# harvardinformatics/IMCoalHMM

Measured on AMD Instinct MI355X. Metric: alignment columns/sec (forward pass), 20-state isolation HMM, higher is better.
Workload: dtype f64

## Files before the change

imcoalhmm_amd/csrc/imcoal_fwd.hip:

```cpp
#include <hip/hip_runtime.h>

#include <algorithm>
#include <cerrno>
#include <climits>
#include <cmath>
#include <cstdint>
#include <cstdio>
#include <cstdlib>
#include <cstring>
#include <list>
#include <atomic>
#include <chrono>
#include <map>
#include <set>
#include <memory>
#include <mutex>
#include <condition_variable>
#include <string>
#include <vector>

#include <unistd.h>

#include "../../include/imcoal_fwd.h"
#include "kernels_plain.hpp"
// ... 35 lines not shown
constexpr size_t DICT_TRAIN_MIN = 32768;
constexpr size_t DICT_TRAIN_MAX = 8u << 20;
constexpr size_t DICT_WIDE_TRAIN_TOKENS = 1u << 19;
constexpr int DICT_MAX_DEPTH = 0;
constexpr size_t DICT_WIDE_MIN_COUNT = 6;
constexpr size_t CTAB_BUDGET = (size_t)24 << 30;
#ifndef IMC_HYBRID_MAX_ALPHABET
#define IMC_HYBRID_MAX_ALPHABET 4096
#endif
constexpr int HYBRID_MAX_ALPHABET = IMC_HYBRID_MAX_ALPHABET;
constexpr size_t Z2GRAN = 4;
constexpr size_t R1_MIN_SEGLEN = 1024;
constexpr size_t R1_MIN_HEAD = 256;
constexpr double R1_HEAD_COLUMNS = 65536.0;
constexpr double R1_HEAD_MIN_COLUMNS = 8192.0;
constexpr int R1_MAX_ROUNDS = 24;
constexpr double R1_DENSE_COLUMNS = 1.0e5;

hipError_t dev_alloc(void **p, size_t bytes);
void dev_free(void *p);

struct DictDev {
    imc::PairDict dict;
    uint16_t *d_left = nullptr, *d_right = nullptr;
    uint16_t *d_order = nullptr;
    std::vector<uint16_t> order;
    std::vector<int> depth;
    uint64_t trained_on = 0;
    pid_t pid = 0;
    ~DictDev()
    {
        if (pid == getpid()) { dev_free(d_left); dev_free(d_right); dev_free(d_order); }
    }
};

struct Ev3 { hipEvent_t a, b, c; };

struct Ctx {
    pid_t pid = 0;
    int device = -1;
    bool ready = false;
    hipStream_t stream = nullptr;
    int cus = 256;
    uint64_t next_obs_id = 1, next_dict_id = 1;
    size_t seg_override = 0;
    int compression = 1;
    int kernel_pref = 0;
    bool profile = false;
    bool rank1_handoff = true;
    int blocked_variant = 4;
    int z4_stream = -1;
    bool table_pairs = true;
    int table_triples = -1;
    bool xcd_affine = true;
    int fuse_tail = 1;
    bool fuse_head = true;
    bool pack_table = true;
    bool guard = false;
    bool use_graphs = false;
    std::vector<Ev3> events;
    std::map<int, std::shared_ptr<DictDev>> dicts;
    uint64_t last_plan[8] = {0, 0, 0, 0, 0, 0, 0, 0};
    uint64_t r1_checked = 0, r1_collapsed = 0;
    std::string last_kernels;
} g;

void drop_plans();
void reset_kernel_attributes();

int ensure_ctx()
{
    const pid_t me = getpid();
    if (g.ready && g.pid == me) return IMC_OK;
    if (g.ready && g.pid != me)
        return fail(IMC_ERR_HIP, "libimcoal_fwd was initialised in the parent process before fork(): fork the chain "
                                 "processes before the first imc_* call of the parent, or use the spawn start method");
    int n = 0;
    if (hipGetDeviceCount(&n) != hipSuccess || n <= 0)
        return fail(IMC_ERR_NODEVICE, "no HIP device available (libimcoal_fwd has no CPU fallback)");
    if (g.device < 0) {
        int cur = 0;
        if (hipGetDevice(&cur) != hipSuccess) cur = 0;
        g.device = cur;
    }
    if (g.device >= n) return fail(IMC_ERR_NODEVICE, "requested device index out of range");
    HIP_TRY(hipSetDevice(g.device));
    hipDeviceProp_t prop;
    HIP_TRY(hipGetDeviceProperties(&prop, g.device));
    if (std::strncmp(prop.gcnArchName, "gfx950", 6) != 0)
        return fail(IMC_ERR_NODEVICE, std::string("device is ") + prop.gcnArchName + ", this library is built for gfx950 only");
    g.cus = prop.multiProcessorCount > 0 ? prop.multiProcessorCount : 256;
    HIP_TRY(hipStreamCreateWithFlags(&g.stream, hipStreamNonBlocking));
    g.use_graphs = std::getenv("IMC_GRAPH") != nullptr;
    if (const char *gd = std::getenv("IMC_GUARD")) g.guard = std::atoi(gd) != 0;
    if (const char *bv = std::getenv("IMC_BLOCKED")) { const int v = std::atoi(bv); if (v >= 2 && v <= 5) g.blocked_variant = v; }
    if (const char *r1 = std::getenv("IMC_RANK1")) g.rank1_handoff = std::atoi(r1) != 0;
    if (const char *pt = std::getenv("IMC_PACK_TABLE")) g.pack_table = std::atoi(pt) != 0;
    if (const char *tp = std::getenv("IMC_TABLE_PAIRS")) g.table_pairs = std::atoi(tp) != 0;
    if (const char *fh = std::getenv("IMC_FUSE_HEAD")) g.fuse_head = std::atoi(fh) != 0;
    if (const char *tt = std::getenv("IMC_TABLE_TRIPLES")) g.table_triples = std::atoi(tt) != 0 ? 1 : 0;
    if (const char *ft = std::getenv("IMC_FUSE_TAIL")) g.fuse_tail = std::max(0, std::min(2, std::atoi(ft)));
    if (const char *xa = std::getenv("IMC_XCD_AFFINE")) g.xcd_affine = std::atoi(xa) != 0;
    if (const char *zs = std::getenv("IMC_Z4_STREAM")) { const int v = std::atoi(zs); if (v >= -1 && v <= 1) g.z4_stream = v; }
    g.pid = me;
    g.ready = true;
    return IMC_OK;
}

struct GuardRec { hipDeviceptr_t va; size_t va_size; hipMemGenericAllocationHandle_t handle; hipDeviceptr_t map; size_t map_size; };
std::map<void *, GuardRec> &g_guard = *new std::map<void *, GuardRec>();

hipError_t dev_alloc(void **p, size_t bytes)
{
    bytes = std::max<size_t>(bytes, 16);
    if (!g.guard) return hipMalloc(p, bytes);
    hipMemAllocationProp prop{};
    prop.type = hipMemAllocationTypePinned;
    prop.location.type = hipMemLocationTypeDevice;
    prop.location.id = g.device;
    size_t gran = 0;
    hipError_t e = hipMemGetAllocationGranularity(&gran, &prop, hipMemAllocationGranularityMinimum);
    if (e != hipSuccess || gran == 0) return e != hipSuccess ? e : hipErrorUnknown;
    GuardRec r{};
    r.map_size = (bytes + gran - 1) / gran * gran;
    r.va_size = r.map_size + 2 * gran;
    e = hipMemAddressReserve(&r.va, r.va_size, gran, nullptr, 0);
    if (e != hipSuccess) return e;
    e = hipMemCreate(&r.handle, r.map_size, &prop, 0);
    if (e != hipSuccess) { (void)hipMemAddressFree(r.va, r.va_size); return e; }
    r.map = (hipDeviceptr_t)((char *)r.va + gran);
    e = hipMemMap(r.map, r.map_size, 0, r.handle, 0);
    if (e == hipSuccess) {
        hipMemAccessDesc ad{};
        ad.location = prop.location;
        ad.flags = hipMemAccessFlagsProtReadWrite;
        e = hipMemSetAccess(r.map, r.map_size, &ad, 1);
        if (e != hipSuccess) (void)hipMemUnmap(r.map, r.map_size);
    }
    if (e != hipSuccess) { (void)hipMemRelease(r.handle); (void)hipMemAddressFree(r.va, r.va_size); return e; }
    void *user = (char *)r.map + (r.map_size - (bytes + 15) / 16 * 16);
    g_guard[user] = r;
    *p = user;
    return hipSuccess;
}

void dev_free(void *p)
{
    if (!p) return;
    auto it = g_guard.find(p);
    if (it == g_guard.end()) { (void)hipFree(p); return; }
    (void)hipDeviceSynchronize();
    (void)hipMemUnmap(it->second.map, it->second.map_size);
// ... 183 lines not shown
    for (int l = 0; l < imc::kNumLevels; ++l) { o->d_tok[l] = nullptr; o->wide[l] = false; o->ntok[l] = 0; o->alphabet[l] = nsym; }
    hipError_t e = wide_raw ? upload_padded(reinterpret_cast<const uint8_t *>(host16), L * sizeof(imc::tok_t), &o->d_sym)
                            : upload_padded(host, L, &o->d_sym);
    if (e != hipSuccess) {
        delete o;
        return fail(e == hipErrorOutOfMemory ? IMC_ERR_OOM : IMC_ERR_HIP,
                    std::string("observation upload: ") + hipGetErrorString(e));
    }
    if (zipped) {
        if (int rc = install_encoding(o, dd, enc)) {
            obs_release(o);
            delete o;
            return rc;
        }
    }
    *out = o;
    return IMC_OK;
}


using ChainFn = void (*)(const ChainDesc *, int, const uint32_t *, uint32_t, uint32_t, const double *, const int *,
                         const int *, uint32_t, double *, int *, double *, int);

struct KernelChoice {
    int R, G, NP, VPW, minw;
    void (*plain)(PropArgs);
    void (*zip)(PropArgs);
    size_t (*zip_lds)(int);
    ChainFn chain;
    bool zip_attr_set;
    void (*big_table_raw)(BigArgs);
    void (*big_table_level)(BigArgs, const uint16_t *, int);
    void (*big_prop)(BigArgs, const BigBlock *);
    int big_prop_waves;
    void (*big_vec)(BigArgs, const BigBlock *, int, int);
    void (*big_vec_tail)(BigArgs, const BigBlock *, int, int);
    int big_vec_waves;
    int big_nslab;
    size_t big_lds;
    void (*zip2)(BigArgs);
    size_t (*zip2_lds)(int);
    bool zip2_attr_set;
    bool plain_attr_set = false;
    void (*zip3)(BigArgs) = nullptr;
    size_t (*zip3_lds)(int) = nullptr;
    bool zip3_attr_set = false;
    void (*zip4)(BigArgs) = nullptr;
    void (*zip4w)(BigArgs) = nullptr;
    void (*zip4s)(BigArgs) = nullptr, (*zip4sw)(BigArgs) = nullptr;
    void (*zip4_raw)(BigArgs) = nullptr;
    void (*zip4_level)(BigArgs, int, int) = nullptr;
    void (*zip4_level2)(BigArgs, const int4 *, int, int, const double *) = nullptr;
    void (*zip4_level2_first)(BigArgs, const int4 *, int, int, const double *) = nullptr;
    void (*zip4_level3)(BigArgs, const int4 *, int, int, const double *) = nullptr;
    void (*zip4_level3_first)(BigArgs, const int4 *, int, int, const double *) = nullptr;
    size_t (*zip4_level3_lds)(size_t) = nullptr;
    size_t (*zip4_lds)(int, int) = nullptr;
    int (*zip4_max_hot)(int, size_t) = nullptr;
    int tok_doubles = 0;
    bool chain_self_emax = false;
    bool zip4_attr_set = false, zip4w_attr_set = false, zip4s_attr_set = false, zip4sw_attr_set = false, zip4_attr_l3 = false;
    bool use3() const;
    size_t blocked_lds(int A) const { return use3() ? zip3_lds(A) : zip2_lds(A); }
};

template <int R, int G, int MW>
KernelChoice make_kc()
{
    constexpr int NP = R * G;
    KernelChoice k{R, G, NP, 64 / G, MW, k_propagate<R, G, MW>, k_zpropagate<R, G>, &ZipGeom<R, G>::lds_bytes,
                   k_chain<NP, (NP <= 12 ? 6 : NP <= 24 ? 4 : NP <= 32 ? 3 : NP <= 64 ? 2 : 1)>, false, nullptr, nullptr, nullptr, 0, nullptr, nullptr, 0, 0, 0, nullptr, nullptr, false};
    k.chain_self_emax = true;
    if constexpr (NP % 4 == 0 && NP <= 24) {
        k.zip2 = k_zpropagate2<NP / 4>;
        k.zip2_lds = &Zip2Geom<NP / 4>::lds_bytes;
        k.zip3 = k_zpropagate3<NP / 4>;
        k.zip3_lds = &Zip3Geom<NP / 4>::lds_bytes;
        k.tok_doubles = Zip3Geom<NP / 4>::TOK;
        if constexpr (NP <= 24) {
            k.zip4 = k_zpropagate4<NP / 4, false, true>;
            k.zip4w = k_zpropagate4<NP / 4, true, true>;
            k.zip4s = k_zpropagate4<NP / 4, false, false>;
            k.zip4sw = k_zpropagate4<NP / 4, true, false>;
            k.zip4_raw = k_z4_raw<NP / 4>;
            k.zip4_level = k_z4_level<NP / 4>;
            k.zip4_level2 = k_z4_level2<NP / 4, false>;
            k.zip4_level2_first = k_z4_level2<NP / 4, true>;
            k.zip4_level3 = k_z4_level3<NP / 4, false>;
            k.zip4_level3_first = k_z4_level3<NP / 4, true>;
            k.zip4_level3_lds = &Z4L3Geom<NP / 4>::lds_bytes;
            k.zip4_lds = &Zip4Geom<NP / 4>::lds_bytes;
            k.zip4_max_hot = &Zip4Geom<NP / 4>::max_hot;
        }
    }
    return k;
}

template <int NT, int NSLAB>
KernelChoice make_big()
{
    constexpr int NP = 16 * NT;
    constexpr bool dealt = NT > 4 && NT % 4 != 0;
    void (*prop)(BigArgs, const BigBlock *) = k_big_propagate<NT, NSLAB>;
    if constexpr (dealt) prop = k_big_propagate_s<NT, NSLAB>;
    return KernelChoice{0, NT, NP, 0, 1, nullptr, nullptr, nullptr, k_chain<NP, 0>, false, k_big_table_raw<NT>,
                        k_big_table_level<NT>, prop, dealt ? BS_WAVES : NT, k_big_vector<NT, false>, k_big_vector<NT, true>, BigVec<NT>::WAVES, NSLAB,
                        BigSlab<NT, NSLAB>::bytes, nullptr, nullptr, false};
}

bool KernelChoice::use3() const { return zip3 && g.blocked_variant >= 3; }

KernelChoice kChoices[] = {
    make_kc<4, 1, 2>(), make_kc<4, 2, 2>(), make_kc<4, 3, 2>(), make_kc<4, 4, 2>(), make_kc<4, 5, 2>(),
    make_kc<3, 8, 2>(), make_kc<2, 14, 2>(), make_kc<2, 16, 2>(), make_kc<2, 20, 1>(), make_kc<1, 48, 1>(),
    make_kc<1, 56, 1>(), make_kc<1, 64, 1>(),
    make_big<6, 1>(), make_big<7, 1>(), make_big<8, 2>(), make_big<9, 3>(), make_big<10, 2>(), make_big<12, 3>(), make_big<14, 7>(),
    make_big<16, 8>(),
};
constexpr int IMC_MAX_N = 256;

KernelChoice kMidChoices[] = {make_big<2, 1>(), make_big<3, 1>(), make_big<4, 1>()};

KernelChoice *choose_kernel(int N, bool prefer_gemm)
{
    if (prefer_gemm && N > 24 && N <= 64)
        for (auto &k : kMidChoices)
            if (k.NP >= N) return &k;
    for (auto &k : kChoices)
        if (k.NP >= N) return &k;
    return nullptr;
}

void reset_kernel_attributes()
{
    for (auto &k : kChoices) k.zip4_attr_l3 = k.zip_attr_set = k.zip2_attr_set = k.zip3_attr_set = k.zip4_attr_set = k.zip4w_attr_set = k.zip4s_attr_set = k.zip4sw_attr_set = k.plain_attr_set = false;
    for (auto &k : kMidChoices) k.zip4_attr_l3 = k.zip_attr_set = k.zip2_attr_set = k.zip3_attr_set = k.zip4_attr_set = k.zip4w_attr_set = k.zip4s_attr_set = k.zip4sw_attr_set = k.plain_attr_set = false;
}


struct Group {
// ... 937 lines not shown
    for (int b = 0; b < B; ++b) {
        double *pp = p->h_params[p->slot] + (size_t)b * p->pstride;
        std::memset(pp, 0, p->pstride * 8);
        const double *pi = pis + (size_t)b * N, *T = Ts + (size_t)b * N * N, *E = Es + (size_t)b * N * S;
        for (int i = 0; i < N; ++i) pp[i] = pi[i];
        double *Tp = pp + NP;
        for (int j = 0; j < N; ++j) std::memcpy(Tp + (size_t)j * NP, T + (size_t)j * N, (size_t)N * 8);
        double *Et = pp + NP + (size_t)NP * NP;
        for (int s = 0; s < S; ++s)
            for (int i = 0; i < N; ++i) Et[(size_t)s * NP + i] = E[(size_t)i * S + s];
    }
    return IMC_OK;
}

int enqueue(Plan *p, hipStream_t stream, double *out, bool allow_tail = true)
{
    KernelChoice *kc = p->kc;
    const int N = p->N, S = p->S, NP = kc->NP, B = p->B;
    hipStreamCaptureStatus cap = hipStreamCaptureStatusNone;
    (void)hipStreamIsCapturing(stream, &cap);
    if (cap == hipStreamCaptureStatusNone && p->have_last && p->last_stream != stream)
        HIP_TRY(hipStreamWaitEvent(stream, p->ev_params[p->last_slot], 0));
    const size_t pbytes = (size_t)B * p->pstride * 8;
    bool fuse_head = false, direct_params = false;
    {
        int active = 0;
        const Group *only = nullptr;
        for (const Group &gr : p->groups)
            if (gr.n_vecs) { ++active; only = &gr; }
        const size_t head_lds = p->pstride * 8;
        fuse_head = g.fuse_head && active == 1 && only->zip4 && g.table_pairs && only->d_tab_desc2 && !only->tab2.empty() &&
                    kc->zip4_level2_first && pbytes <= STAGE_KERNEL_MAX_BYTES && head_lds <= 16 * 1024;
        direct_params = g.fuse_head && active == 1 && only->zip2 && !only->zip4 && kc->use3() && pbytes <= STAGE_KERNEL_MAX_BYTES &&
                        only->blocks.size() * (size_t)B <= 32 && p->pstride * 8 <= 8192 &&
                        ((kc->blocked_lds(only->A) + 15) & ~(size_t)15) + p->pstride * 8 <= LDS_BUDGET;
    }
    if (fuse_head || direct_params) {
    } else if (pbytes <= STAGE_KERNEL_MAX_BYTES) {
        const unsigned n2 = (unsigned)(pbytes / 16);
        hipLaunchKernelGGL(k_stage_params, dim3((n2 + 255) / 256), dim3(256), 0, stream,
                           reinterpret_cast<const double2 *>(p->h_params_dev[p->slot]), reinterpret_cast<double2 *>(p->d_params), n2);
        HIP_TRY(hipGetLastError());
    } else {
        HIP_TRY(hipMemcpyAsync(p->d_params, p->h_params[p->slot], pbytes, hipMemcpyHostToDevice, stream));
    }

    uint64_t *lp = p->lp;
    lp[0] = p->n_segs; lp[1] = p->n_vecs; lp[2] = lp[3] = lp[4] = lp[5] = lp[6] = lp[7] = 0;
    Ev3 ev{nullptr, nullptr, nullptr};
    const bool prof = g.profile && p->n_vecs;
    bool a_recorded = false;
    if (prof) { HIP_TRY(hipEventCreate(&ev.a)); HIP_TRY(hipEventCreate(&ev.b)); HIP_TRY(hipEventCreate(&ev.c)); }
#define IMC_MARK_A() do { if (prof && !a_recorded) { HIP_TRY(hipEventRecord(ev.a, stream)); a_recorded = true; } } while (0)
    bool tail_used = false;
    p->kernels.clear();
    auto note = [&](const std::string &k) { p->kernels += (p->kernels.empty() ? "" : "+") + k; };
    for (const Group &gr : p->groups) {
        if (!gr.n_vecs) continue;
        if (!gr.zip4) IMC_MARK_A();
        const std::string strm = gr.zip ? "[tokens]" : "[columns]";
        PropArgs a;
        a.segs = p->d_segs; a.vecs = p->d_vecs + gr.vec_begin; a.n_vecs = gr.n_vecs; a.vec_base = gr.vec_begin;
        a.n_vecs_total = p->n_vecs; a.N = N; a.S = S;
        a.params = p->d_params; a.pstride = p->pstride; a.P = p->levels[0].d_P; a.EX = p->levels[0].d_EX;
        a.A = gr.A; a.tok_left = gr.zip ? gr.dict->d_left : nullptr; a.tok_right = gr.zip ? gr.dict->d_right : nullptr;
        if (gr.big) {
            BigArgs ba;
            ba.n_phases = 0;
            ba.tail = nullptr; ba.tailX = nullptr; ba.tailE = nullptr; ba.tail_arrive = nullptr; ba.tail_out = nullptr; ba.tail_stride = 0; ba.n_chunks = p->n_chunks;
            ba.segs = p->d_segs; ba.seg_ids = gr.d_seg_ids; ba.seg_vec0 = gr.d_seg_out; ba.blocks = nullptr;
            ba.n_group_segs = (uint32_t)gr.seg_ids.size(); ba.n_vecs_total = p->n_vecs;
            ba.N = N; ba.S = S; ba.A = gr.A; ba.params = p->d_params; ba.params_src = nullptr; ba.pstride = p->pstride; ba.PP = NP;
            ba.tok_left = gr.zip ? gr.dict->d_left : nullptr; ba.tok_right = gr.zip ? gr.dict->d_right : nullptr;
            ba.Ctab = gr.d_Ctab; ba.cex = gr.d_cex;
            ba.Cpack = gr.d_Cpack; ba.TS = N + (N & 1);
            ba.P = p->levels[0].d_P; ba.EX = p->levels[0].d_EX;
            ba.phase = gr.rank1 ? 1 : 0; ba.t_from = 0; ba.t_to = gr.rank1 ? gr.checkpoints[0] : INT_MAX;
            ba.r1flag = gr.d_r1flag; ba.r1at = gr.d_r1at; ba.r1u = gr.d_r1u;
            ba.r1alpha = gr.d_r1alpha; ba.n_segs = p->n_segs;
            ba.tab_order = nullptr; ba.tab_lvl = nullptr; ba.tab_nlvl = 0; ba.hot = nullptr; ba.n_hot = 0; ba.tab_desc = nullptr;
            if (gr.rank1) HIP_TRY(hipMemsetAsync(gr.d_r1flag, 0, (size_t)B * p->n_segs * 4, stream));
            hipLaunchKernelGGL(kc->big_table_raw, dim3((unsigned)S, (unsigned)B), dim3(kc->G * 64), 0, stream, ba);
            HIP_TRY(hipGetLastError());
            if (gr.zip) {
                const DictDev &dd = *gr.dict;
                size_t i0 = 0;
                while (i0 < dd.order.size()) {
                    size_t i1 = i0;
                    while (i1 < dd.order.size() && dd.depth[dd.order[i1]] == dd.depth[dd.order[i0]]) ++i1;
                    size_t r0 = i0;
                    while (r0 < i1) {
                        while (r0 < i1 && (int)dd.order[r0] >= gr.A) ++r0;
                        size_t r1 = r0;
                        while (r1 < i1 && (int)dd.order[r1] < gr.A) ++r1;
                        if (r1 > r0) {
                            hipLaunchKernelGGL(kc->big_table_level, dim3((unsigned)(r1 - r0), (unsigned)B), dim3(kc->G * 64), 0,
                                               stream, ba, (const uint16_t *)dd.d_order, (int)r0);
                            HIP_TRY(hipGetLastError());
                        }
                        r0 = r1;
                    }
                    i0 = i1;
                }
            }
            if (gr.bigvec) {
                const unsigned grid = B >= 8 ? 8u * (unsigned)gr.big_blocks.size() * (unsigned)((B + 7) / 8)
// ... 30 lines not shown
                                           (const BigBlock *)gr.d_tail_blocks, (int)gr.tail_blocks.size(), B);
                        HIP_TRY(hipGetLastError());
                    }
                    hipLaunchKernelGGL(kc->big_prop, dim3((unsigned)gr.big_blocks.size(), (unsigned)B), dim3(kc->big_prop_waves * 64), kc->big_lds,
                                       stream, ba, (const BigBlock *)gr.d_big_blocks);
                }
                note("rank1-handoff");
            }
            if (gr.zip) { lp[4] = gr.seglen; lp[5] += gr.vsteps * (uint64_t)B; lp[6] += gr.stream_len; lp[7] = std::max(lp[7], (uint64_t)gr.A); }
            else { lp[2] = gr.seglen; lp[3] += gr.vsteps * (uint64_t)B; }
        } else if (gr.zip2) {
            BigArgs ba;
            ba.n_phases = 0;
            ba.tail = nullptr; ba.tailX = nullptr; ba.tailE = nullptr; ba.tail_arrive = nullptr; ba.tail_out = nullptr; ba.tail_stride = 0; ba.n_chunks = p->n_chunks;
            ba.segs = p->d_segs; ba.seg_ids = nullptr; ba.seg_vec0 = nullptr; ba.blocks = gr.d_blocks;
            ba.n_group_segs = (uint32_t)gr.blocks.size(); ba.n_vecs_total = p->n_vecs;
            ba.N = N; ba.S = S; ba.A = gr.A; ba.params = p->d_params; ba.params_src = nullptr; ba.pstride = p->pstride; ba.PP = NP;
            ba.tok_left = gr.zip ? gr.dict->d_left : nullptr; ba.tok_right = gr.zip ? gr.dict->d_right : nullptr;
            ba.Ctab = nullptr; ba.cex = nullptr; ba.Cpack = nullptr; ba.TS = 0;
            ba.P = p->levels[0].d_P; ba.EX = p->levels[0].d_EX;
            ba.tab_order = gr.d_tab_order; ba.tab_lvl = gr.d_tab_lvl; ba.tab_nlvl = gr.tab_nlvl;
            ba.hot = gr.d_hot; ba.n_hot = gr.n_hot; ba.tab_desc = gr.d_tab_desc;
            if (gr.d_tails && (g.fuse_tail == 2 || (g.fuse_tail == 1 && gr.tail_stride <= 4)) && allow_tail && kc->use3()) {
                ba.tail = gr.d_tails; ba.tailX = gr.d_tailX; ba.tailE = gr.d_tailE; ba.tail_arrive = gr.d_tail_arrive;
                ba.tail_out = out; ba.tail_stride = gr.tail_stride; ba.n_chunks = p->n_chunks;
                tail_used = true;
            }
            if (gr.zip4) {
                ba.Ctab = gr.d_Ctab; ba.cex = gr.d_cex;
                if (!fuse_head) {
                    hipLaunchKernelGGL(kc->zip4_raw, dim3((unsigned)S + 1, (unsigned)B), dim3(256), 0, stream, ba);
                    HIP_TRY(hipGetLastError());
                }
                if (g.table_pairs && (g.table_triples == 1 || (g.table_triples < 0 && NP <= 12)) && gr.d_tab_desc3) {
                    bool head = fuse_head;
                    if (!kc->zip4_attr_l3) {
                        HIP_TRY(hipFuncSetAttribute((const void *)kc->zip4_level3, hipFuncAttributeMaxDynamicSharedMemorySize, (int)LDS_BUDGET));
                        HIP_TRY(hipFuncSetAttribute((const void *)kc->zip4_level3_first, hipFuncAttributeMaxDynamicSharedMemorySize, (int)LDS_BUDGET));
                        kc->zip4_attr_l3 = true;
                    }
                    for (const auto &lc : gr.tab3) {
                        const dim3 grid((unsigned)(lc.second + Z4L3_WAVES - 1) / Z4L3_WAVES, (unsigned)B);
                        if (head)
                            hipLaunchKernelGGL(kc->zip4_level3_first, grid, dim3(Z4L3_WAVES * 64), kc->zip4_level3_lds(p->pstride), stream, ba,
                                               (const int4 *)gr.d_tab_desc3, lc.first, lc.second, (const double *)p->h_params_dev[p->slot]);
                        else
                            hipLaunchKernelGGL(kc->zip4_level3, grid, dim3(Z4L3_WAVES * 64), kc->zip4_level3_lds(0), stream, ba,
                                               (const int4 *)gr.d_tab_desc3, lc.first, lc.second, (const double *)nullptr);
                        head = false;
                        HIP_TRY(hipGetLastError());
                    }
                } else if (g.table_pairs && gr.d_tab_desc2) {
                    bool head = fuse_head;
                    for (const auto &lc : gr.tab2) {
                        if (head)
                            hipLaunchKernelGGL(kc->zip4_level2_first, dim3((unsigned)(lc.second + 3) / 4, (unsigned)B), dim3(64),
                                               p->pstride * 8, stream, ba,
                                               (const int4 *)gr.d_tab_desc2, lc.first, lc.second, (const double *)p->h_params_dev[p->slot]);
                        else
                            hipLaunchKernelGGL(kc->zip4_level2, dim3((unsigned)(lc.second + 3) / 4, (unsigned)B), dim3(64), 0, stream, ba,
                                               (const int4 *)gr.d_tab_desc2, lc.first, lc.second, (const double *)nullptr);
                        head = false;
                        HIP_TRY(hipGetLastError());
                    }
                } else
                for (int d = 0; d < gr.tab_nlvl; ++d) {
                    const int first = gr.tab_lvl[d], count = gr.tab_lvl[d + 1] - first;
                    hipLaunchKernelGGL(kc->zip4_level, dim3((unsigned)(count + 3) / 4, (unsigned)B), dim3(64), 0, stream, ba, first, count);
                    HIP_TRY(hipGetLastError());
                }
                void (*scan)(BigArgs) = gr.stream_table ? (gr.wide_tokens ? kc->zip4sw : kc->zip4s) : (gr.wide_tokens ? kc->zip4w : kc->zip4);
                bool &attr4 = gr.stream_table ? (gr.wide_tokens ? kc->zip4sw_attr_set : kc->zip4s_attr_set)
                                              : (gr.wide_tokens ? kc->zip4w_attr_set : kc->zip4_attr_set);
                if (!attr4) {
                    HIP_TRY(hipFuncSetAttribute((const void *)scan, hipFuncAttributeMaxDynamicSharedMemorySize, (int)LDS_BUDGET));
                    attr4 = true;
                }
                IMC_MARK_A();
                dim3 scan_grid(ba.n_group_segs, (unsigned)B);
                if (g.xcd_affine && B > 1) {
                    int first = 0, wg = 0;
                    auto phase = [&](int sets, int n_sets_total) {
                        ba.ph_begin[ba.n_phases] = wg; ba.ph_first[ba.n_phases] = first; ba.ph_sets[ba.n_phases] = sets;
                        ++ba.n_phases;
                        const int nb = (int)ba.n_group_segs;
                        wg += sets >= 8 ? 8 * nb * (n_sets_total / 8) : 8 * ((nb + 8 / sets - 1) / (8 / sets));
                        first += n_sets_total;
                    };
                    if (B >= 8) phase(8, B / 8 * 8);
                    for (int sets : {4, 2, 1})
                        if ((B % 8) & sets) phase(sets, sets);
                    scan_grid = dim3((unsigned)wg);
                }
                hipLaunchKernelGGL(scan, scan_grid, dim3(Z2WAVES * 64), kc->zip4_lds(gr.A, gr.n_hot), stream, ba);
                note(std::string("k_zpropagate4<") + std::to_string(NP / 4) + (gr.wide_tokens ? ",16" : "") + (gr.stream_table ? ",streamed>" : ">") + strm);
                lp[4] = gr.seglen; lp[5] += gr.vsteps * (uint64_t)B; lp[6] += gr.stream_len; lp[7] = std::max(lp[7], (uint64_t)gr.A);
                HIP_TRY(hipGetLastError());
                continue;
            }
            const bool v3 = kc->use3();
            bool &attr_set = v3 ? kc->zip3_attr_set : kc->zip2_attr_set;
            if (!attr_set) {
                HIP_TRY(hipFuncSetAttribute((const void *)(v3 ? kc->zip3 : kc->zip2), hipFuncAttributeMaxDynamicSharedMemorySize,
                                            (int)LDS_BUDGET));
                attr_set = true;
            }
            size_t lds3 = kc->blocked_lds(gr.A);
            if (direct_params) { ba.params_src = p->h_params_dev[p->slot]; lds3 = ((lds3 + 15) & ~(size_t)15) + p->pstride * 8; }
            hipLaunchKernelGGL(v3 ? kc->zip3 : kc->zip2, dim3(ba.n_group_segs, (unsigned)B), dim3(Z2WAVES * 64), lds3, stream, ba);
            note(std::string(v3 ? "k_zpropagate3<" : "k_zpropagate2<") + std::to_string(NP / 4) + ">" + strm);
            if (gr.zip) { lp[4] = gr.seglen; lp[5] += gr.vsteps * (uint64_t)B; lp[6] += gr.stream_len; lp[7] = std::max(lp[7], (uint64_t)gr.A); }
            else { lp[2] = gr.seglen; lp[3] += gr.vsteps * (uint64_t)B; }
        } else if (gr.zip) {
            const size_t lds = kc->zip_lds(gr.A);
            if (!kc->zip_attr_set) {
                HIP_TRY(hipFuncSetAttribute((const void *)kc->zip, hipFuncAttributeMaxDynamicSharedMemorySize,
                                            (int)LDS_BUDGET));
                kc->zip_attr_set = true;
            }
            const uint32_t vpb = (uint32_t)(ZWAVES * kc->VPW);
            dim3 grid((gr.n_vecs + vpb - 1) / vpb, (unsigned)B);
            hipLaunchKernelGGL(kc->zip, grid, dim3(ZWAVES * 64), lds, stream, a);
            note("k_zpropagate<" + std::to_string(kc->R) + "," + std::to_string(kc->G) + ">" + strm);
            lp[4] = gr.seglen; lp[5] += gr.vsteps * (uint64_t)B; lp[6] += gr.stream_len; lp[7] = std::max(lp[7], (uint64_t)gr.A);
        } else {
            const uint32_t vpb = (uint32_t)(WPB * kc->VPW);
            dim3 grid((gr.n_vecs + vpb - 1) / vpb, (unsigned)B);
            const size_t lds = ((size_t)WPB * kc->VPW * NP + (size_t)S * NP) * 8;
            if (lds > LDS_BUDGET) return fail(IMC_ERR_ARG, "emission table (S x N) too large for LDS");
            if (lds > 48 * 1024 && !kc->plain_attr_set) {
                HIP_TRY(hipFuncSetAttribute((const void *)kc->plain, hipFuncAttributeMaxDynamicSharedMemorySize,
                                            (int)LDS_BUDGET));
                kc->plain_attr_set = true;
            }
            hipLaunchKernelGGL(kc->plain, grid, dim3(WPB * 64), lds, stream, a);
            note("k_propagate<" + std::to_string(kc->R) + "," + std::to_string(kc->G) + ">" + strm);
            lp[2] = gr.seglen; lp[3] += gr.vsteps * (uint64_t)B;
        }
        HIP_TRY(hipGetLastError());
    }
    IMC_MARK_A();
#undef IMC_MARK_A
    if (prof) HIP_TRY(hipEventRecord(ev.b, stream));
    if (tail_used) note("fused-tail");
    for (size_t l = 0; l + 1 < p->levels.size() && !tail_used; ++l) {
        const Level &in = p->levels[l], &ot = p->levels[l + 1];
        if (!in.n_segs || !ot.n_chains) continue;
        if (!kc->chain_self_emax) {
            hipLaunchKernelGGL(k_emax, dim3((in.n_segs + 255) / 256, (unsigned)B), dim3(256), 0, stream,
                               in.d_vec0, in.d_first, in.n_segs, in.n_vecs, N, in.d_EX, in.d_EMAX);
            HIP_TRY(hipGetLastError());
        }
        const int threads = (int)round_up((size_t)NP, 64);
        const bool last_level = l + 2 == p->levels.size();
        hipLaunchKernelGGL(kc->chain, dim3(ot.n_chains, (unsigned)B), dim3(threads), 0, stream,
                           ot.d_chains, N, in.d_vec0, in.n_segs, in.n_vecs, in.d_P, in.d_EX, in.d_EMAX,
                           ot.n_vecs, ot.d_P, ot.d_EX, (last_level && p->finish_fused) ? out : (double *)nullptr, p->n_chunks);
        HIP_TRY(hipGetLastError());
    }
    if (p->n_chunks && !p->finish_fused && !tail_used) {
        const Level &last = p->levels.back();
        hipLaunchKernelGGL(k_finish, dim3((p->n_chunks + 63) / 64, (unsigned)B), dim3(64), 0, stream,
                           p->d_final_vec, p->n_chunks, N, NP, last.n_vecs, last.d_P, last.d_EX, out);
        HIP_TRY(hipGetLastError());
    }
    if (prof) {
        HIP_TRY(hipEventRecord(ev.c, stream));
        g.events.push_back(ev);
    }
    if (cap == hipStreamCaptureStatusNone) {
        HIP_TRY(hipEventRecord(p->ev_params[p->slot], stream));
        p->ev_used[p->slot] = true;
        p->last_stream = stream;
        p->last_slot = p->slot;
        p->have_last = true;
    }
    return IMC_OK;
}

void collect_rank1_stats(Plan *p)
{
    g.r1_checked = g.r1_collapsed = 0;
    for (Group &gr : p->groups) {
        if (!gr.rank1 || gr.r1_segs.empty() || gr.checkpoints.empty()) continue;
        std::vector<int> flags((size_t)p->B * p->n_segs);
        if (hipMemcpy(flags.data(), gr.d_r1flag, flags.size() * 4, hipMemcpyDeviceToHost) != hipSuccess) continue;
        for (int b = 0; b < p->B; ++b)
            for (const auto &sl : gr.r1_segs) {
                if ((int)sl.second <= gr.checkpoints[0]) continue;
                ++g.r1_checked;
                g.r1_collapsed += flags[(size_t)b * p->n_segs + sl.first] ? 1 : 0;
            }
        if (getenv("IMC_DEBUG_R1")) {
            std::vector<int> at((size_t)p->B * p->n_segs);
            if (hipMemcpy(at.data(), gr.d_r1at, at.size() * 4, hipMemcpyDeviceToHost) != hipSuccess) continue;
            std::map<int, int> hist;
// ... 608 lines not shown
```

imcoalhmm_amd/csrc/kernels_zip4.hpp:

```cpp
#pragma once
#include "kernels_zip3.hpp"

template <int NT>
struct Zip4Geom {
    using G3 = Zip3Geom<NT>;
    static constexpr int TOK = G3::TOK;
    static constexpr int slots(int H) { return (H + 1 > Z2SLOTS + 1 ? H + 1 : Z2SLOTS + 1); }
    static constexpr size_t lds_bytes(int A, int H) { return (size_t)slots(H) * TOK * 8 + (size_t)(2 * (A + 2) + 64) * 4 + 16; }
    static constexpr int max_hot(int A, size_t budget)
    {
        const size_t fixed = (size_t)(2 * (A + 2) + 64) * 4 + 16;
        const size_t n = budget > fixed ? (budget - fixed) / ((size_t)TOK * 8) : 0;
        return n > 1 ? (int)n - 1 : 0;
    }
};

template <int NT>
__device__ __forceinline__ void zip4_step_regs(const double (&Pin)[NT][NT], double (&Pout)[NT][NT], const double (&Areg)[NT][NT])
{
#pragma unroll
    for (int I = 0; I < NT; ++I)
#pragma unroll
        for (int K = 0; K < NT; ++K)
#pragma unroll
// ... 20 lines not shown
{
    using Geo = Zip3Geom<NT>;
    constexpr int NP = Geo::NP, TOK = Geo::TOK;
    const int b = blockIdx.y, sidx = blockIdx.x;
    const double *pp = a.params + (size_t)b * a.pstride;
    const double *Tp = pp + a.PP;
    const double *Etg = pp + a.PP + (size_t)a.PP * a.PP;
    double *Gt = a.Ctab + (size_t)b * (a.A + 1) * TOK;
    int *Gc = a.cex + (size_t)b * (a.A + 1);
    const int entry = sidx < a.S ? sidx : a.A;
    for (int idx = threadIdx.x; idx < NP * NP; idx += blockDim.x) {
        const int i = idx / NP, j = idx - i * NP;
        Gt[(size_t)entry * TOK + Geo::idx(i, j)] = sidx < a.S ? Etg[(size_t)sidx * a.PP + i] * Tp[(size_t)j * a.PP + i] : (i == j ? 1.0 : 0.0);
    }
    if (threadIdx.x == 0) Gc[entry] = 0;
}

template <int NT>
__global__ __launch_bounds__(64) void k_z4_level(BigArgs a, int first, int count)
{
    using Geo = Zip3Geom<NT>;
    constexpr int TOK = Geo::TOK;
    const int b = blockIdx.y, lane = threadIdx.x;
    const int q = lane >> 4, bq = (lane >> 2) & 3, r = lane & 3;
    const int lo = (q * 4 + r) * Geo::NTE, lx = q * 4 + r;
    double *Gt = a.Ctab + (size_t)b * (a.A + 1) * TOK;
    int *Gc = a.cex + (size_t)b * (a.A + 1);
    const int ti = blockIdx.x * 4 + bq;
    const bool have = ti < count;
    const int4 td = have ? a.tab_desc[first + ti] : make_int4(a.A, a.A, a.A, 0);
    const int z = td.x, zl = td.y, zr = td.z;
    const double *Gl = Gt + (size_t)zl * TOK, *Gr = Gt + (size_t)zr * TOK;
    double Bt[NT][NT], Ar[NT][NT], Out[NT][NT];
#pragma unroll
    for (int K = 0; K < NT; ++K)
#pragma unroll
        for (int J = 0; J < NT; ++J) Bt[K][J] = Gl[Geo::idx(4 * K + q, 4 * J + r)];
#pragma unroll
    for (int I = 0; I < NT; ++I) zip4_load_row_global<NT>(Ar[I], Gr, I, lo, lx);
    const int cel = Gc[zl], cer = Gc[zr];
    zip4_step_regs<NT>(Bt, Out, Ar);
    int e2 = 0;
    zip3_rescale<NT>(Out, e2);
    if (have) {
        double *Gz = Gt + (size_t)z * TOK;
#pragma unroll
        for (int K = 0; K < NT; ++K)
#pragma unroll
            for (int J = 0; J < NT; ++J) Gz[Geo::idx(4 * K + q, 4 * J + r)] = Out[K][J];
        if (q == 0 && r == 0) Gc[z] = cel + cer + e2;
    }
}

template <int NT, bool FIRST>
__global__ __launch_bounds__(64) void k_z4_level2(BigArgs a, const int4 *desc2, int first, int count, const double *params_src)
{
    using Geo = Zip3Geom<NT>;
    constexpr int TOK = Geo::TOK, NP = Geo::NP;
    __shared__ __attribute__((aligned(16))) double turn[4 * TOK];
    extern __shared__ __attribute__((aligned(16))) double rawtab[];
    const int b = blockIdx.y, lane = threadIdx.x;
    const int q = lane >> 4, bq = (lane >> 2) & 3, r = lane & 3;
    const int lo = (q * 4 + r) * Geo::NTE, lx = q * 4 + r;
    double *Gt = a.Ctab + (size_t)b * (a.A + 1) * TOK;
    int *Gc = a.cex + (size_t)b * (a.A + 1);
    const int IDENT = a.A;
    if constexpr (FIRST) {
        const double *src = params_src + (size_t)b * a.pstride;
        double *lp = rawtab;
        for (int k0 = 0; k0 < (int)a.pstride; k0 += 8 * 128) {
            double2 v[8];
#pragma unroll
            for (int u = 0; u < 8; ++u) {
                const int k = k0 + u * 128 + lane * 2;
                v[u] = k < (int)a.pstride ? *reinterpret_cast<const double2 *>(src + k) : make_double2(0.0, 0.0);
            }
#pragma unroll
            for (int u = 0; u < 8; ++u) {
                const int k = k0 + u * 128 + lane * 2;
                if (k < (int)a.pstride) *reinterpret_cast<double2 *>(lp + k) = v[u];
            }
        }
        wave_fence();
        if (blockIdx.x == 0) {
            double *dp = const_cast<double *>(a.params) + (size_t)b * a.pstride;
            for (int k = lane * 2; k < (int)a.pstride; k += 128) *reinterpret_cast<double2 *>(dp + k) = *reinterpret_cast<const double2 *>(lp + k);
        }
        const double *Tp = lp + a.PP, *Etg = lp + a.PP + (size_t)a.PP * a.PP;
        for (int s = blockIdx.x; s <= a.S; s += gridDim.x) {
            double *Gz = Gt + (size_t)(s < a.S ? s : IDENT) * TOK;
            for (int idx = lane; idx < NP * NP; idx += 64) {
                const int i = idx / NP, j = idx - i * NP;
                Gz[Geo::idx(i, j)] = s < a.S ? Etg[(size_t)s * a.PP + i] * Tp[(size_t)j * a.PP + i] : (i == j ? 1.0 : 0.0);
            }
            if (lane == 0) Gc[s < a.S ? s : IDENT] = 0;
        }
    }
    const int ti = blockIdx.x * 4 + bq;
    int4 d0 = ti < count ? desc2[2 * (first + ti)] : make_int4(-1, 0, 0, 0);
    int4 d1 = ti < count ? desc2[2 * (first + ti) + 1] : make_int4(0, 0, 0, 0);
    const bool have = d0.x >= 0;
    if (!have) { d0 = make_int4(IDENT, IDENT, IDENT, 0); d1 = make_int4(IDENT, IDENT, IDENT, IDENT); }
    const int z = d0.x, zl = d0.y, zr = d0.z;
    const bool needL = (d0.w & 1) != 0, needR = (d0.w & 2) != 0;
    const bool anyL = __any(needL), anyR = __any(needR);

    const double *lp = rawtab;
    auto leaf = [&](int tok, int i, int j) __attribute__((always_inline)) {
        const double *Tp = lp + a.PP, *Etg = lp + a.PP + (size_t)a.PP * a.PP;
        const double v = Etg[(size_t)(tok == IDENT ? 0 : tok) * a.PP + i] * Tp[(size_t)j * a.PP + i];
        return tok == IDENT ? (i == j ? 1.0 : 0.0) : v;
    };
    auto expo = [&](int tok) __attribute__((always_inline)) { if constexpr (FIRST) return 0; else return Gc[tok]; };
    auto load_B = [&](double (&Bt)[NT][NT], int tok) __attribute__((always_inline)) {
        const double *G = Gt + (size_t)tok * TOK;
#pragma unroll
        for (int K = 0; K < NT; ++K)
#pragma unroll
            for (int J = 0; J < NT; ++J) {
                if constexpr (FIRST) Bt[K][J] = leaf(tok, 4 * K + q, 4 * J + r);
                else Bt[K][J] = G[Geo::idx(4 * K + q, 4 * J + r)];
            }
    };
    auto load_A = [&](double (&Ar)[NT][NT], int tok) __attribute__((always_inline)) {
        const double *G = Gt + (size_t)tok * TOK;
#pragma unroll
        for (int I = 0; I < NT; ++I) {
            if constexpr (FIRST) {
#pragma unroll
                for (int K = 0; K < NT; ++K) Ar[I][K] = leaf(tok, 4 * I + r, 4 * K + q);
            } else zip4_load_row_global<NT>(Ar[I], G, I, lo, lx);
        }
    };

    double L[NT][NT];
    int eL;
    if (anyL) {
        const int t0 = needL ? d1.x : zl, t1 = needL ? d1.y : IDENT;
        double Bt[NT][NT], Ar[NT][NT];
        load_B(Bt, t0);
        load_A(Ar, t1);
        eL = expo(t0) + expo(t1);
        zip4_step_regs<NT>(Bt, L, Ar);
    } else {
        load_B(L, zl);
        eL = expo(zl);
    }
    double R[NT][NT];
    int eR;
// ... 445 lines not shown
```

Before: 382.2 billion.

## Add split table-pair kernel assigning one table entry per wave for small levels

```diff
diff --git a/imcoalhmm_amd/csrc/imcoal_fwd.hip b/imcoalhmm_amd/csrc/imcoal_fwd.hip
--- a/imcoalhmm_amd/csrc/imcoal_fwd.hip
+++ b/imcoalhmm_amd/csrc/imcoal_fwd.hip
@@ -111,6 +111,8 @@
     int z4_stream = -1;
     bool table_pairs = true;
     int table_triples = -1;
+    bool table_split = true;
+    int table_split_max = -1;
     bool xcd_affine = true;
     int fuse_tail = 1;
     bool fuse_head = true;
@@ -157,6 +159,8 @@
     if (const char *pt = std::getenv("IMC_PACK_TABLE")) g.pack_table = std::atoi(pt) != 0;
     if (const char *tp = std::getenv("IMC_TABLE_PAIRS")) g.table_pairs = std::atoi(tp) != 0;
     if (const char *fh = std::getenv("IMC_FUSE_HEAD")) g.fuse_head = std::atoi(fh) != 0;
+    if (const char *ts = std::getenv("IMC_TABLE_SPLIT")) g.table_split = std::atoi(ts) != 0;
+    if (const char *tm = std::getenv("IMC_TABLE_SPLIT_MAX")) g.table_split_max = std::max(0, std::atoi(tm));
     if (const char *tt = std::getenv("IMC_TABLE_TRIPLES")) g.table_triples = std::atoi(tt) != 0 ? 1 : 0;
     if (const char *ft = std::getenv("IMC_FUSE_TAIL")) g.fuse_tail = std::max(0, std::min(2, std::atoi(ft)));
     if (const char *xa = std::getenv("IMC_XCD_AFFINE")) g.xcd_affine = std::atoi(xa) != 0;
@@ -446,6 +450,8 @@
     void (*zip4_level)(BigArgs, int, int) = nullptr;
     void (*zip4_level2)(BigArgs, const int4 *, int, int, const double *) = nullptr;
     void (*zip4_level2_first)(BigArgs, const int4 *, int, int, const double *) = nullptr;
+    void (*zip4_level2_split)(BigArgs, const int4 *, int, int, const double *) = nullptr;
+    void (*zip4_level2_split_first)(BigArgs, const int4 *, int, int, const double *) = nullptr;
     void (*zip4_level3)(BigArgs, const int4 *, int, int, const double *) = nullptr;
     void (*zip4_level3_first)(BigArgs, const int4 *, int, int, const double *) = nullptr;
     size_t (*zip4_level3_lds)(size_t) = nullptr;
@@ -480,6 +486,8 @@
             k.zip4_level = k_z4_level<NP / 4>;
             k.zip4_level2 = k_z4_level2<NP / 4, false>;
             k.zip4_level2_first = k_z4_level2<NP / 4, true>;
+            k.zip4_level2_split = k_z4_level2<NP / 4, false, Z4_SPLIT_WAVES>;
+            k.zip4_level2_split_first = k_z4_level2<NP / 4, true, Z4_SPLIT_WAVES_FIRST>;
             k.zip4_level3 = k_z4_level3<NP / 4, false>;
             k.zip4_level3_first = k_z4_level3<NP / 4, true>;
             k.zip4_level3_lds = &Z4L3Geom<NP / 4>::lds_bytes;
@@ -1523,6 +1531,7 @@
     bool a_recorded = false;
     if (prof) { HIP_TRY(hipEventCreate(&ev.a)); HIP_TRY(hipEventCreate(&ev.b)); HIP_TRY(hipEventCreate(&ev.c)); }
 #define IMC_MARK_A() do { if (prof && !a_recorded) { HIP_TRY(hipEventRecord(ev.a, stream)); a_recorded = true; } } while (0)
+    bool split_used = false;
     bool tail_used = false;
     p->kernels.clear();
     auto note = [&](const std::string &k) { p->kernels += (p->kernels.empty() ? "" : "+") + k; };
@@ -1659,8 +1668,19 @@
                     }
                 } else if (g.table_pairs && gr.d_tab_desc2) {
                     bool head = fuse_head;
+                    const size_t split_max = g.table_split_max >= 0 ? (size_t)g.table_split_max : (size_t)4 * g.cus;
                     for (const auto &lc : gr.tab2) {
-                        if (head)
+                        if (g.table_split && (size_t)lc.second * B <= split_max) {
+                            if (head)
+                                hipLaunchKernelGGL(kc->zip4_level2_split_first, dim3((unsigned)(lc.second + Z4_SPLIT_WAVES_FIRST - 1) / Z4_SPLIT_WAVES_FIRST, (unsigned)B),
+                                                   dim3(Z4_SPLIT_WAVES_FIRST * 64), p->pstride * 8, stream, ba,
+                                                   (const int4 *)gr.d_tab_desc2, lc.first, lc.second, (const double *)p->h_params_dev[p->slot]);
+                            else
+                                hipLaunchKernelGGL(kc->zip4_level2_split, dim3((unsigned)(lc.second + Z4_SPLIT_WAVES - 1) / Z4_SPLIT_WAVES, (unsigned)B),
+                                                   dim3(Z4_SPLIT_WAVES * 64), 0, stream, ba,
+                                                   (const int4 *)gr.d_tab_desc2, lc.first, lc.second, (const double *)nullptr);
+                            split_used = true;
+                        } else if (head)
                             hipLaunchKernelGGL(kc->zip4_level2_first, dim3((unsigned)(lc.second + 3) / 4, (unsigned)B), dim3(64),
                                                p->pstride * 8, stream, ba,
                                                (const int4 *)gr.d_tab_desc2, lc.first, lc.second, (const double *)p->h_params_dev[p->slot]);
@@ -1749,6 +1769,7 @@
     IMC_MARK_A();
 #undef IMC_MARK_A
     if (prof) HIP_TRY(hipEventRecord(ev.b, stream));
+    if (split_used) note("table-split");
     if (tail_used) note("fused-tail");
     for (size_t l = 0; l + 1 < p->levels.size() && !tail_used; ++l) {
         const Level &in = p->levels[l], &ot = p->levels[l + 1];
diff --git a/imcoalhmm_amd/csrc/kernels_zip4.hpp b/imcoalhmm_amd/csrc/kernels_zip4.hpp
--- a/imcoalhmm_amd/csrc/kernels_zip4.hpp
+++ b/imcoalhmm_amd/csrc/kernels_zip4.hpp
@@ -96,49 +96,187 @@
     }
 }
 
-template <int NT, bool FIRST>
-__global__ __launch_bounds__(64) void k_z4_level2(BigArgs a, const int4 *desc2, int first, int count, const double *params_src)
+template <int NT, bool FIRST, bool NL, bool NR>
+__device__ __forceinline__ void z4_split_entry(const BigArgs &a, double *Gt, int *Gc, double *turn, const double *lp,
+                                               int z, int zl, int zr, int ll, int lr, int rl, int rr)
 {
     using Geo = Zip3Geom<NT>;
-    constexpr int TOK = Geo::TOK, NP = Geo::NP;
-    __shared__ __attribute__((aligned(16))) double turn[4 * TOK];
+    constexpr int TOK = Geo::TOK, NPASS = (NT + 3) / 4;
+    const int lane = threadIdx.x & 63;
+    const int q = lane >> 4, bq = (lane >> 2) & 3, r = lane & 3;
+    const int lo = (q * 4 + r) * Geo::NTE, lx = q * 4 + r;
+    const int IDENT = a.A;
+    int tcol[NPASS], toff[NPASS], tstr[NPASS];
+    bool tv[NPASS];
+#pragma unroll
+    for (int p = 0; p < NPASS; ++p) {
+        const int J = bq + 4 * p;
+        tv[p] = J < NT;
+        const int Jc = tv[p] ? J : 0;
+        const bool mainp = Jc < Geo::NTE;
+        tcol[p] = 4 * Jc + r;
+        toff[p] = mainp ? (r * 4 + q) * Geo::NTE + Jc : Geo::MAIN + r * 4 + q;
+        tstr[p] = mainp ? 16 * Geo::NTE : 16;
+    }
+    auto leaf = [&](int tok, int i, int j) __attribute__((always_inline)) {
+        const double *Tp = lp + a.PP, *Etg = lp + a.PP + (size_t)a.PP * a.PP;
+        const double v = Etg[(size_t)(tok == IDENT ? 0 : tok) * a.PP + i] * Tp[(size_t)j * a.PP + i];
+        return tok == IDENT ? (i == j ? 1.0 : 0.0) : v;
+    };
+    auto expo = [&](int tok) __attribute__((always_inline)) { if constexpr (FIRST) return 0; else return Gc[tok]; };
+    auto load_B = [&](double (&Bt)[NPASS][NT], int tok) __attribute__((always_inline)) {
+        const double *G = Gt + (size_t)tok * TOK;
+#pragma unroll
+        for (int p = 0; p < NPASS; ++p)
+#pragma unroll
+            for (int K = 0; K < NT; ++K) {
+                if constexpr (FIRST) Bt[p][K] = leaf(tok, 4 * K + q, tcol[p]);
+                else Bt[p][K] = G[toff[p] + K * tstr[p]];
+            }
+    };
+    auto load_A = [&](double (&Ar)[NT][NT], int tok) __attribute__((always_inline)) {
+        const double *G = Gt + (size_t)tok * TOK;
+#pragma unroll
+        for (int I = 0; I < NT; ++I) {
+            if constexpr (FIRST) {
+#pragma unroll
+                for (int K = 0; K < NT; ++K) Ar[I][K] = leaf(tok, 4 * I + r, 4 * K + q);
+            } else zip4_load_row_global<NT>(Ar[I], G, I, lo, lx);
+        }
+    };
+    auto product = [&](const double (&Bt)[NPASS][NT], double (&Out)[NPASS][NT], const double (&Ar)[NT][NT]) __attribute__((always_inline)) {
+#pragma unroll
+        for (int K = 0; K < NT; ++K)
+#pragma unroll
+            for (int p = 0; p < NPASS; ++p)
+#pragma unroll
+                for (int I = 0; I < NT; ++I)
+                    Out[p][I] = __builtin_amdgcn_mfma_f64_4x4x4f64(Ar[I][K], Bt[p][K], K == 0 ? 0.0 : Out[p][I], 0, 0, 0);
+    };
+
+    double LB[NPASS][NT], LA[NT][NT], RB[NPASS][NT], RA[NT][NT];
+    int eL, eR;
+    if constexpr (NL) { load_B(LB, ll); load_A(LA, lr); eL = expo(ll) + expo(lr); }
+    else { load_B(LB, zl); eL = expo(zl); }
+    if constexpr (NR) { load_B(RB, rl); load_A(RA, rr); eR = expo(rl) + expo(rr); }
+    else { load_A(RA, zr); eR = expo(zr); }
+    double L[NPASS][NT];
+    if constexpr (NL) product(LB, L, LA);
+    else {
+#pragma unroll
+        for (int p = 0; p < NPASS; ++p)
+#pragma unroll
+            for (int K = 0; K < NT; ++K) L[p][K] = LB[p][K];
+    }
+    double R[NT][NT];
+    if constexpr (NR) {
+        double Rt[NPASS][NT];
+        product(RB, Rt, RA);
+#pragma unroll
+        for (int p = 0; p < NPASS; ++p)
+#pragma unroll
+            for (int I = 0; I < NT; ++I)
+                if (tv[p]) turn[toff[p] + I * tstr[p]] = Rt[p][I];
+        wave_fence();
+#pragma unroll
+        for (int I = 0; I < NT; ++I) zip3_load_row<NT>(R[I], turn, I, lo, lx);
+    } else {
+#pragma unroll
+        for (int I = 0; I < NT; ++I)
+#pragma unroll
+            for (int K = 0; K < NT; ++K) R[I][K] = RA[I][K];
+    }
+    double Out[NPASS][NT];
+    product(L, Out, R);
+    int hmax = 0;
+#pragma unroll
+    for (int p = 0; p < NPASS; ++p)
+#pragma unroll
+        for (int I = 0; I < NT; ++I) hmax = max(hmax, tv[p] ? __double2hiint(Out[p][I]) & 0x7fffffff : 0);
+    const int field = hmax >> 20;
+    int e = field == 0 ? INT_MIN : field == 0x7ff ? INT_MAX : field - 1022;
+#pragma unroll
+    for (int m = 1; m <= 32; m *= 2) e = max(e, __shfl_xor(e, m, 64));
+    e = (e == INT_MAX || e == INT_MIN) ? 0 : e;
+    double *Gz = Gt + (size_t)z * TOK;
+#pragma unroll
+    for (int p = 0; p < NPASS; ++p)
+#pragma unroll
+        for (int I = 0; I < NT; ++I)
+            if (tv[p]) Gz[toff[p] + I * tstr[p]] = ldexp(Out[p][I], -e);
+    if (lane == 0) Gc[z] = eL + eR + e;
+}
+
+constexpr int Z4_SPLIT_WAVES = 1;
+constexpr int Z4_SPLIT_WAVES_FIRST = 4;
+template <int NT, bool FIRST, int SPLIT = 0>
+__global__ __launch_bounds__((SPLIT ? SPLIT : 1) * 64) void k_z4_level2(BigArgs a, const int4 *desc2, int first, int count, const double *params_src)
+{
+    using Geo = Zip3Geom<NT>;
+    constexpr int TOK = Geo::TOK, NP = Geo::NP, WAVES = SPLIT ? SPLIT : 1, THREADS = WAVES * 64;
+    __shared__ __attribute__((aligned(16))) double turn[(SPLIT ? WAVES : 4) * TOK];
     extern __shared__ __attribute__((aligned(16))) double rawtab[];
-    const int b = blockIdx.y, lane = threadIdx.x;
+    const int b = blockIdx.y, tid = threadIdx.x, lane = tid & 63;
     const int q = lane >> 4, bq = (lane >> 2) & 3, r = lane & 3;
     const int lo = (q * 4 + r) * Geo::NTE, lx = q * 4 + r;
     double *Gt = a.Ctab + (size_t)b * (a.A + 1) * TOK;
     int *Gc = a.cex + (size_t)b * (a.A + 1);
     const int IDENT = a.A;
+    const int wti = blockIdx.x * WAVES + (tid >> 6);
+    int4 e0 = make_int4(-1, 0, 0, 0), e1 = make_int4(0, 0, 0, 0);
+    if constexpr (SPLIT != 0) {
+        if (wti < count) { e0 = desc2[2 * (first + wti)]; e1 = desc2[2 * (first + wti) + 1]; }
+    }
+    auto publish = [&]() __attribute__((always_inline)) {
+        const double *lp = rawtab;
+        if (blockIdx.x == 0) {
+            double *dp = const_cast<double *>(a.params) + (size_t)b * a.pstride;
+            for (int k = tid * 2; k < (int)a.pstride; k += 2 * THREADS) *reinterpret_cast<double2 *>(dp + k) = *reinterpret_cast<const double2 *>(lp + k);
+        }
+        const double *Tp = lp + a.PP, *Etg = lp + a.PP + (size_t)a.PP * a.PP;
+        for (int s = blockIdx.x; s <= a.S; s += gridDim.x) {
+            double *Gz = Gt + (size_t)(s < a.S ? s : IDENT) * TOK;
+            for (int idx = tid; idx < NP * NP; idx += THREADS) {
+                const int i = idx / NP, j = idx - i * NP;
+                Gz[Geo::idx(i, j)] = s < a.S ? Etg[(size_t)s * a.PP + i] * Tp[(size_t)j * a.PP + i] : (i == j ? 1.0 : 0.0);
+            }
+            if (tid == 0) Gc[s < a.S ? s : IDENT] = 0;
+        }
+    };
     if constexpr (FIRST) {
         const double *src = params_src + (size_t)b * a.pstride;
         double *lp = rawtab;
-        for (int k0 = 0; k0 < (int)a.pstride; k0 += 8 * 128) {
+        for (int k0 = 0; k0 < (int)a.pstride; k0 += 8 * 2 * THREADS) {
             double2 v[8];
 #pragma unroll
             for (int u = 0; u < 8; ++u) {
-                const int k = k0 + u * 128 + lane * 2;
+                const int k = k0 + (u * THREADS + tid) * 2;
                 v[u] = k < (int)a.pstride ? *reinterpret_cast<const double2 *>(src + k) : make_double2(0.0, 0.0);
             }
 #pragma unroll
             for (int u = 0; u < 8; ++u) {
-                const int k = k0 + u * 128 + lane * 2;
+                const int k = k0 + (u * THREADS + tid) * 2;
                 if (k < (int)a.pstride) *reinterpret_cast<double2 *>(lp + k) = v[u];
             }
         }
-        wave_fence();
-        if (blockIdx.x == 0) {
-            double *dp = const_cast<double *>(a.params) + (size_t)b * a.pstride;
-            for (int k = lane * 2; k < (int)a.pstride; k += 128) *reinterpret_cast<double2 *>(dp + k) = *reinterpret_cast<const double2 *>(lp + k);
-        }
-        const double *Tp = lp + a.PP, *Etg = lp + a.PP + (size_t)a.PP * a.PP;
-        for (int s = blockIdx.x; s <= a.S; s += gridDim.x) {
-            double *Gz = Gt + (size_t)(s < a.S ? s : IDENT) * TOK;
-            for (int idx = lane; idx < NP * NP; idx += 64) {
-                const int i = idx / NP, j = idx - i * NP;
-                Gz[Geo::idx(i, j)] = s < a.S ? Etg[(size_t)s * a.PP + i] * Tp[(size_t)j * a.PP + i] : (i == j ? 1.0 : 0.0);
-            }
-            if (lane == 0) Gc[s < a.S ? s : IDENT] = 0;
-        }
+        if constexpr (WAVES > 1) __syncthreads();
+        else wave_fence();
+        if constexpr (SPLIT == 0) publish();
+    }
+    if constexpr (SPLIT != 0) {
+        const int z = __builtin_amdgcn_readfirstlane(e0.x);
+        if (z >= 0) {
+            const int zl = __builtin_amdgcn_readfirstlane(e0.y), zr = __builtin_amdgcn_readfirstlane(e0.z), fl = __builtin_amdgcn_readfirstlane(e0.w);
+            const int ll = __builtin_amdgcn_readfirstlane(e1.x), lr = __builtin_amdgcn_readfirstlane(e1.y);
+            const int rl = __builtin_amdgcn_readfirstlane(e1.z), rr = __builtin_amdgcn_readfirstlane(e1.w);
+            double *mine = turn + (size_t)(tid >> 6) * TOK;
+            if (fl == 3) z4_split_entry<NT, FIRST, true, true>(a, Gt, Gc, mine, rawtab, z, zl, zr, ll, lr, rl, rr);
+            else if (fl == 2) z4_split_entry<NT, FIRST, false, true>(a, Gt, Gc, mine, rawtab, z, zl, zr, ll, lr, rl, rr);
+            else if (fl == 1) z4_split_entry<NT, FIRST, true, false>(a, Gt, Gc, mine, rawtab, z, zl, zr, ll, lr, rl, rr);
+            else z4_split_entry<NT, FIRST, false, false>(a, Gt, Gc, mine, rawtab, z, zl, zr, ll, lr, rl, rr);
+        }
+        if constexpr (FIRST) publish();
+        return;
     }
     const int ti = blockIdx.x * 4 + bq;
     int4 d0 = ti < count ? desc2[2 * (first + ti)] : make_int4(-1, 0, 0, 0);
```

After: 396.4 billion, median of 6. +3.7%, better.
